# can-lehmann/exprgrad

Measured on AMD Instinct MI355X. Metric: GFLOP/s matmul 4096^3 f32 (1 GPU), higher is better.
Workload: dtype f32

## Files before the change

exprgrad_amd/csrc/kernels/gemm_split_bf16.hip:

```cpp
#include <algorithm>
#include <cfloat>

#include "gemm_fused.hpp"
#include "../eg_internal.hpp"
#include "../switches.hpp"

namespace {

typedef __bf16 bf16x8 __attribute__((ext_vector_type(8)));
typedef float f32x4 __attribute__((ext_vector_type(4)));


struct SplitOperand {
  const float* src;
  long ld;
  long R;
  int kc;
  __bf16* dst;
};

__device__ __forceinline__ void unit_coords(const SplitOperand& o, long K, long u, long& r, long& chunk) {
  const long cpr = K / 8, t = u >> 6;
  const int l = (int)(u & 63);
  if (o.kc) {
    const long per = cpr / 4;
    r = (t / per) * 16 + (l >> 2);
    chunk = (t % per) * 4 + (l & 3);
  } else {
    const long per = cpr / 2;
    r = (t / per) * 32 + (l >> 1);
    chunk = (t % per) * 2 + (l & 1);
  }
}

__device__ __forceinline__ void load_unit(const SplitOperand& o, long r, long chunk, float (&x)[8]) {
  if (o.kc) {
    const f32x4* p = reinterpret_cast<const f32x4*>(o.src + r * o.ld + chunk * 8);
    const f32x4 v0 = __builtin_nontemporal_load(p), v1 = __builtin_nontemporal_load(p + 1);
#pragma unroll
    for (int j = 0; j < 4; ++j) {
      x[j] = v0[j];
      x[4 + j] = v1[j];
    }
  } else {
    const float* p = o.src + chunk * 8 * o.ld + r;
#pragma unroll
    for (int j = 0; j < 8; ++j) x[j] = __builtin_nontemporal_load(p + j * o.ld);
  }
}

__device__ __forceinline__ void split_unit(const SplitOperand& o, long K, long r, long chunk, const float (&x)[8], bool& bad) {
  bf16x8 h0, h1, h2;
#pragma unroll
  for (int j = 0; j < 8; ++j) {
    const float v = x[j];
    const __bf16 b0 = (__bf16)v;
    const float r1 = v - (float)b0;
    const __bf16 b1 = (__bf16)r1;
    const float f1 = (float)b1;
    const float r2 = r1 - f1;
    const __bf16 b2 = (__bf16)r2;
    const float f2 = (float)b2;
    bad |= !(r2 == f2);
    bad |= v != 0.f && __builtin_fabsf(v) < FLT_MIN;
    bad |= (f1 != 0.f && __builtin_fabsf(f1) < FLT_MIN) || (f2 != 0.f && __builtin_fabsf(f2) < FLT_MIN);
    h0[j] = b0;
    h1[j] = b1;
    h2[j] = b2;
  }
  const long plane = o.R * K;
  bf16x8* d = reinterpret_cast<bf16x8*>(o.dst + ((chunk >> 1) * o.R + r) * 16 + (chunk & 1) * 8);
  const long ps = plane / 8;
  d[0] = h0;
  d[ps] = h1;
  d[2 * ps] = h2;
}

constexpr int SPLIT_NT = 256;
constexpr int SPLIT_U = 2;

__global__ __launch_bounds__(SPLIT_NT) void split_planes_kernel(SplitOperand a, SplitOperand b, long K, long units_a, long units,
                                                              unsigned* flag, unsigned epoch) {
  constexpr long STEP = (long)SPLIT_NT * SPLIT_U;
  const long per = ((units + gridDim.x - 1) / gridDim.x + STEP - 1) / STEP * STEP;
  const long lo = (long)blockIdx.x * per, hi = lo + per < units ? lo + per : units;
  bool bad = false;
  for (long base = lo; base < hi; base += STEP) {
    float x[SPLIT_U][8];
    long r[SPLIT_U], c[SPLIT_U];
#pragma unroll
    for (int i = 0; i < SPLIT_U; ++i) {
      const long u = base + i * SPLIT_NT + threadIdx.x;
      if (u >= hi) continue;
      const bool in_a = u < units_a;
      unit_coords(in_a ? a : b, K, in_a ? u : u - units_a, r[i], c[i]);
      load_unit(in_a ? a : b, r[i], c[i], x[i]);
    }
#pragma unroll
    for (int i = 0; i < SPLIT_U; ++i) {
      const long u = base + i * SPLIT_NT + threadIdx.x;
      if (u >= hi) continue;
      split_unit(u < units_a ? a : b, K, r[i], c[i], x[i], bad);
    }
  }
  if (__builtin_expect(bad, 0)) *(volatile unsigned*)flag = epoch;
}


constexpr int BM = 256, BN = 256, WM = 128, WN = 64, NT = 512;
constexpr int STAGES = 3;
constexpr int PLANE_BYTES = BM * 16 * 2;
constexpr int STAGE_BYTES = 6 * PLANE_BYTES;
constexpr int LOADS = STAGE_BYTES / (NT * 16);

struct SplitGemmArgs {
  const __bf16* pa;
  const __bf16* pb;
  float* C;
  const float* bias;
  long M, N, K, ldc;
  int tiles_m, tiles_n;
  int accumulate;
  const unsigned* flag;
  unsigned epoch;
};

__device__ __forceinline__ int xcd_remap(int bid, int nwg) {
  constexpr int NXCD = 8;
  const int q = nwg / NXCD, r = nwg % NXCD;
  const int xcd = bid % NXCD, local = bid / NXCD;
  return (xcd < r ? xcd * (q + 1) : r * (q + 1) + (xcd - r) * q) + local;
}
__device__ __forceinline__ void tile_origin(int wgid, int tiles_m, int tiles_n, long& m_blk, long& n_blk) {
  constexpr int GROUP = 8;
  const int per_group = GROUP * tiles_n;
  const int first_m = (wgid / per_group) * GROUP;
  const int gsize = min(tiles_m - first_m, GROUP);
  const int in_group = wgid % per_group;
  m_blk = (long)(first_m + in_group % gsize) * BM;
  n_blk = (long)(in_group / gsize) * BN;
}

__device__ __forceinline__ const void* uniform_ptr(const void* p) {
  const unsigned long v = reinterpret_cast<unsigned long>(p);
  const unsigned lo = __builtin_amdgcn_readfirstlane((unsigned)v), hi = __builtin_amdgcn_readfirstlane((unsigned)(v >> 32));
  return reinterpret_cast<const void*>(((unsigned long)hi << 32) | lo);
}

__global__ __launch_bounds__(NT) void split_gemm_kernel(SplitGemmArgs a) {
  if (*(volatile const unsigned*)a.flag == a.epoch) return;
  __shared__ __attribute__((aligned(16))) unsigned char lds[STAGES * STAGE_BYTES];

  const int tid = threadIdx.x, lane = tid & 63, wave = tid >> 6;
  const int wr = wave >> 2, wc = wave & 3;
  long m_blk, n_blk;
  tile_origin(xcd_remap(blockIdx.x, gridDim.x), a.tiles_m, a.tiles_n, m_blk, n_blk);

  const __amdgpu_buffer_rsrc_t ra = __builtin_amdgcn_make_buffer_rsrc(
      const_cast<void*>(uniform_ptr(a.pa + m_blk * 16)), (short)0, -1, 0x00020000);
  const __amdgpu_buffer_rsrc_t rb = __builtin_amdgcn_make_buffer_rsrc(
      const_cast<void*>(uniform_ptr(a.pb + n_blk * 16)), (short)0, -1, 0x00020000);
  const unsigned a_plane = (unsigned)(a.M * a.K * 2), b_plane = (unsigned)(a.N * a.K * 2);
  const unsigned a_ktile = (unsigned)(a.M * 32), b_ktile = (unsigned)(a.N * 32);
  const unsigned voff = (unsigned)tid * 16;

  auto issue = [&](int kt, int s) {
    unsigned char* st = lds + s * STAGE_BYTES + wave * 1024;
#pragma unroll
    for (int i = 0; i < LOADS; ++i) {
      __attribute__((address_space(3))) void* dst = (__attribute__((address_space(3))) void*)(st + i * PLANE_BYTES);
      if (i < 3)
        __builtin_amdgcn_raw_ptr_buffer_load_lds(ra, dst, 16, voff, (unsigned)i * a_plane + (unsigned)kt * a_ktile, 0, 0);
      else
        __builtin_amdgcn_raw_ptr_buffer_load_lds(rb, dst, 16, voff, (unsigned)(i - 3) * b_plane + (unsigned)kt * b_ktile, 0, 0);
    }
  };

  f32x4 acc[8][4];
#pragma unroll
  for (int i = 0; i < 8; ++i)
#pragma unroll
    for (int j = 0; j < 4; ++j)
#pragma unroll
      for (int r = 0; r < 4; ++r) acc[i][j][r] = 0.f;

  const int sel = lane >> 5;
  const int a_row = (wr * WM + (lane & 15)) * 32 + ((lane >> 4) & 1) * 16;
  const int b_row = 3 * PLANE_BYTES + (wc * WN + (lane & 15)) * 32 + ((lane >> 4) & 1) * 16;
  const int a01_off = a_row + sel * PLANE_BYTES, a02_off = a_row + 2 * sel * PLANE_BYTES;
  const int b21_off = b_row + (2 - sel) * PLANE_BYTES, b10_off = b_row + (1 - sel) * PLANE_BYTES, b00_off = b_row;

  const int KT = (int)(a.K / 16);
  issue(0, 0);
  if (KT > 1) issue(1, 1);
  int s = 0;
  for (int kt = 0; kt < KT; ++kt) {
    if (kt + 1 < KT) asm volatile("s_waitcnt vmcnt(6)" ::: "memory");
    else asm volatile("s_waitcnt vmcnt(0)" ::: "memory");
    __builtin_amdgcn_s_barrier();
    asm volatile("" ::: "memory");
    if (kt + 2 < KT) issue(kt + 2, s == 0 ? 2 : s - 1);
    const unsigned char* st = lds + s * STAGE_BYTES;
    bf16x8 fb21[4], fb10[4], fb00[4];
#pragma unroll
    for (int j = 0; j < 4; ++j) {
      fb21[j] = *reinterpret_cast<const bf16x8*>(st + b21_off + j * 512);
      fb10[j] = *reinterpret_cast<const bf16x8*>(st + b10_off + j * 512);
      fb00[j] = *reinterpret_cast<const bf16x8*>(st + b00_off + j * 512);
    }
#pragma unroll
    for (int i = 0; i < 8; ++i) {
      const bf16x8 fa01 = *reinterpret_cast<const bf16x8*>(st + a01_off + i * 512);
      const bf16x8 fa02 = *reinterpret_cast<const bf16x8*>(st + a02_off + i * 512);
#pragma unroll
      for (int j = 0; j < 4; ++j) acc[i][j] = __builtin_amdgcn_mfma_f32_16x16x32_bf16(fa01, fb21[j], acc[i][j], 0, 0, 0);
#pragma unroll
      for (int j = 0; j < 4; ++j) acc[i][j] = __builtin_amdgcn_mfma_f32_16x16x32_bf16(fa01, fb10[j], acc[i][j], 0, 0, 0);
#pragma unroll
      for (int j = 0; j < 4; ++j) acc[i][j] = __builtin_amdgcn_mfma_f32_16x16x32_bf16(fa02, fb00[j], acc[i][j], 0, 0, 0);
    }
    s = s == STAGES - 1 ? 0 : s + 1;
  }

  __syncthreads();
  float* park = reinterpret_cast<float*>(lds) + wave * 64 * WN;
  const int prow = lane >> 4, pc4 = (lane & 15) * 4;
  const long col = n_blk + wc * WN + pc4;
  f32x4 b4 = {0.f, 0.f, 0.f, 0.f};
  if (a.bias) b4 = *reinterpret_cast<const f32x4*>(a.bias + col);
#pragma unroll
  for (int h = 0; h < 2; ++h) {
#pragma unroll
    for (int i = 0; i < 4; ++i)
#pragma unroll
      for (int j = 0; j < 4; ++j)
#pragma unroll
        for (int r = 0; r < 4; ++r) park[(i * 16 + 4 * prow + r) * WN + j * 16 + (lane & 15)] = acc[4 * h + i][j][r];
    asm volatile("s_waitcnt lgkmcnt(0)" ::: "memory");
#pragma unroll
    for (int q = 0; q < 16; ++q) {
      const int row = 4 * q + prow;
      f32x4 v = *reinterpret_cast<const f32x4*>(park + row * WN + pc4);
      f32x4* c = reinterpret_cast<f32x4*>(a.C + (m_blk + wr * WM + h * 64 + row) * a.ldc + col);
      if (a.accumulate) v = *c + v;
      if (a.bias) v = v + b4;
      *c = v;
    }
    asm volatile("s_waitcnt lgkmcnt(0)" ::: "memory");
  }
}

inline bool aligned16(const void* p) { return (reinterpret_cast<uintptr_t>(p) & 15) == 0; }

constexpr size_t kPlaneCap = 1ull << 30;

}

namespace eg {
namespace gemm {

int sgemm_split(eg_ctx* ctx, int trans_a, int trans_b, long M, long N, long K, const float* A, long lda, const float* B, long ldb,
                float* C, long ldc, int accumulate, const float* bias) {
  if (!ctx || !A || !B || !C || M <= 0 || N <= 0 || K <= 0) return EG_ERR_UNSUPPORTED;
  if (lda < (trans_a ? M : K) || ldb < (trans_b ? K : N) || ldc < N) return EG_ERR_UNSUPPORTED;
  if (eg::sw::on("EG_NO_SPLIT_GEMM")) return EG_ERR_UNSUPPORTED;
  if (M % BM != 0 || N % BN != 0 || K % 32 != 0 || K < 2048) return EG_ERR_UNSUPPORTED;
  if ((M / BM) * (N / BN) < ctx->compute_units) return EG_ERR_UNSUPPORTED;
  const size_t plane_bytes = 6 * (size_t)(M + N) * (size_t)K;
  if (plane_bytes > kPlaneCap || 6 * (size_t)std::max(M, N) * (size_t)K >= (1ull << 31)) return EG_ERR_UNSUPPORTED;
  if (!aligned16(A) || !aligned16(B) || (!trans_a && lda % 4 != 0) || (trans_b && ldb % 4 != 0)) return EG_ERR_UNSUPPORTED;
  if (!aligned16(C) || ldc % 4 != 0 || (bias && !aligned16(bias))) return EG_ERR_UNSUPPORTED;
  if (!exact_single_launch(ctx, trans_a, trans_b, M, N, K, A, lda, B, ldb, C, ldc, bias)) return EG_ERR_UNSUPPORTED;

  int rc = eg::set_device(ctx);
  if (rc) return rc;
  if (!ctx->split_flag) {
    EG_HIP_CHECK(hipMalloc((void**)&ctx->split_flag, sizeof(unsigned)));
    EG_HIP_CHECK(hipMemset(ctx->split_flag, 0, sizeof(unsigned)));
  }
  rc = eg::ensure_workspace(ctx, plane_bytes);
  if (rc) return rc;
  if (++ctx->split_epoch == 0) ctx->split_epoch = 1;
  const unsigned epoch = ctx->split_epoch;

  __bf16* pa = static_cast<__bf16*>(ctx->workspace);
  __bf16* pb = pa + 3 * (size_t)M * K;
  const SplitOperand oa = {A, lda, M, trans_a ? 0 : 1, pa};
  const SplitOperand ob = {B, ldb, N, trans_b ? 1 : 0, pb};
  const long units_a = M * K / 8, units = (M + N) * K / 8;
  long blocks = (units + SPLIT_NT * SPLIT_U - 1) / (SPLIT_NT * SPLIT_U);
  if (blocks > 8L * ctx->compute_units) blocks = 8L * ctx->compute_units;
  hipLaunchKernelGGL(split_planes_kernel, dim3((unsigned)blocks), dim3(SPLIT_NT), 0, ctx->stream, oa, ob, K, units_a, units,
                     ctx->split_flag, epoch);
  EG_HIP_CHECK(hipGetLastError());

  SplitGemmArgs g = {};
  g.pa = pa;
  g.pb = pb;
  g.C = C;
  g.bias = bias;
  g.M = M;
  g.N = N;
  g.K = K;
  g.ldc = ldc;
  g.tiles_m = (int)(M / BM);
  g.tiles_n = (int)(N / BN);
  g.accumulate = accumulate;
  g.flag = ctx->split_flag;
  g.epoch = epoch;
  hipLaunchKernelGGL(split_gemm_kernel, dim3((unsigned)(g.tiles_m * g.tiles_n)), dim3(NT), 0, ctx->stream, g);
  EG_HIP_CHECK(hipGetLastError());

  return sgemm_exact(ctx, trans_a, trans_b, M, N, K, A, lda, B, ldb, C, ldc, accumulate, bias, ctx->split_flag, epoch);
}

}
}
```

Before: 238,400.

## Specialize wave roles in split-bf16 GEMM: half the waves load, others prefetch fragments

Adds a skew mode, on by default. Waves with bit 2 set issue the global-to-LDS loads for themselves and their partner wave. The other waves issue no loads and read the next stage's B and A-head fragments at the end of each iteration, which staggers LDS reads against MFMA work across waves. The A fragment loads inside the inner loop are also software-pipelined one row ahead, and the wave index is forced to be scalar. Skew mode waits for vmcnt(0) every iteration, which may expose load latency, and an optional timestamp instrumentation path is compiled in under a macro.

```diff
diff --git a/exprgrad_amd/csrc/kernels/gemm_split_bf16.hip b/exprgrad_amd/csrc/kernels/gemm_split_bf16.hip
--- a/exprgrad_amd/csrc/kernels/gemm_split_bf16.hip
+++ b/exprgrad_amd/csrc/kernels/gemm_split_bf16.hip
@@ -121,6 +121,7 @@
   long M, N, K, ldc;
   int tiles_m, tiles_n;
   int accumulate;
+  int skew;
   const unsigned* flag;
   unsigned epoch;
 };
@@ -147,11 +148,29 @@
   return reinterpret_cast<const void*>(((unsigned long)hi << 32) | lo);
 }
 
+constexpr int ROLE_LOAD_OWN = 1, ROLE_LOAD_PARTNER = 2, ROLE_READ_TOP = 4, ROLE_READ_AHEAD = 8;
+constexpr int PARTNER = 4;
+
+#ifdef EG_SPLIT_GEMM_STAMPS
+constexpr int STAMP_BLOCKS = 1024;
+__device__ unsigned long long g_split_stamps[STAMP_BLOCKS][8][4];
+#define EG_STAMP(t)                                                                  \
+  do {                                                                               \
+    __builtin_amdgcn_sched_barrier(0);                                               \
+    asm volatile("s_memtime %0\n\ts_waitcnt lgkmcnt(0)" : "=s"(t)::"memory"); \
+    __builtin_amdgcn_sched_barrier(0);                                               \
+  } while (0)
+#else
+#define EG_STAMP(t) \
+  do {              \
+  } while (0)
+#endif
+
 __global__ __launch_bounds__(NT) void split_gemm_kernel(SplitGemmArgs a) {
   if (*(volatile const unsigned*)a.flag == a.epoch) return;
   __shared__ __attribute__((aligned(16))) unsigned char lds[STAGES * STAGE_BYTES];
 
-  const int tid = threadIdx.x, lane = tid & 63, wave = tid >> 6;
+  const int tid = threadIdx.x, lane = tid & 63, wave = __builtin_amdgcn_readfirstlane(tid >> 6);
   const int wr = wave >> 2, wc = wave & 3;
   long m_blk, n_blk;
   tile_origin(xcd_remap(blockIdx.x, gridDim.x), a.tiles_m, a.tiles_n, m_blk, n_blk);
@@ -162,18 +181,23 @@
       const_cast<void*>(uniform_ptr(a.pb + n_blk * 16)), (short)0, -1, 0x00020000);
   const unsigned a_plane = (unsigned)(a.M * a.K * 2), b_plane = (unsigned)(a.N * a.K * 2);
   const unsigned a_ktile = (unsigned)(a.M * 32), b_ktile = (unsigned)(a.N * 32);
-  const unsigned voff = (unsigned)tid * 16;
-
-  auto issue = [&](int kt, int s) {
-    unsigned char* st = lds + s * STAGE_BYTES + wave * 1024;
+  const unsigned voff = (unsigned)lane * 16;
+
+  auto pieces = [&](int kt, int s, int w) {
+    unsigned char* st = lds + s * STAGE_BYTES + w * 1024;
+    const unsigned at = (unsigned)kt * a_ktile + (unsigned)w * 1024, bt = (unsigned)kt * b_ktile + (unsigned)w * 1024;
 #pragma unroll
     for (int i = 0; i < LOADS; ++i) {
       __attribute__((address_space(3))) void* dst = (__attribute__((address_space(3))) void*)(st + i * PLANE_BYTES);
       if (i < 3)
-        __builtin_amdgcn_raw_ptr_buffer_load_lds(ra, dst, 16, voff, (unsigned)i * a_plane + (unsigned)kt * a_ktile, 0, 0);
+        __builtin_amdgcn_raw_ptr_buffer_load_lds(ra, dst, 16, voff, (unsigned)i * a_plane + at, 0, 0);
       else
-        __builtin_amdgcn_raw_ptr_buffer_load_lds(rb, dst, 16, voff, (unsigned)(i - 3) * b_plane + (unsigned)kt * b_ktile, 0, 0);
-    }
+        __builtin_amdgcn_raw_ptr_buffer_load_lds(rb, dst, 16, voff, (unsigned)(i - 3) * b_plane + bt, 0, 0);
+    }
+  };
+  auto issue = [&](int kt, int s, int r) {
+    if (r & ROLE_LOAD_OWN) pieces(kt, s, wave);
+    if (r & ROLE_LOAD_PARTNER) pieces(kt, s, wave ^ PARTNER);
   };
 
   f32x4 acc[8][4];
@@ -190,37 +214,89 @@
   const int a01_off = a_row + sel * PLANE_BYTES, a02_off = a_row + 2 * sel * PLANE_BYTES;
   const int b21_off = b_row + (2 - sel) * PLANE_BYTES, b10_off = b_row + (1 - sel) * PLANE_BYTES, b00_off = b_row;
 
-  const int KT = (int)(a.K / 16);
-  issue(0, 0);
-  if (KT > 1) issue(1, 1);
-  int s = 0;
-  for (int kt = 0; kt < KT; ++kt) {
-    if (kt + 1 < KT) asm volatile("s_waitcnt vmcnt(6)" ::: "memory");
-    else asm volatile("s_waitcnt vmcnt(0)" ::: "memory");
-    __builtin_amdgcn_s_barrier();
-    asm volatile("" ::: "memory");
-    if (kt + 2 < KT) issue(kt + 2, s == 0 ? 2 : s - 1);
-    const unsigned char* st = lds + s * STAGE_BYTES;
-    bf16x8 fb21[4], fb10[4], fb00[4];
+  bf16x8 fb21[4], fb10[4], fb00[4], fa01, fa02;
+  auto read_head = [&](const unsigned char* st) {
 #pragma unroll
     for (int j = 0; j < 4; ++j) {
       fb21[j] = *reinterpret_cast<const bf16x8*>(st + b21_off + j * 512);
       fb10[j] = *reinterpret_cast<const bf16x8*>(st + b10_off + j * 512);
       fb00[j] = *reinterpret_cast<const bf16x8*>(st + b00_off + j * 512);
     }
+    fa01 = *reinterpret_cast<const bf16x8*>(st + a01_off);
+    fa02 = *reinterpret_cast<const bf16x8*>(st + a02_off);
+  };
+#pragma unroll
+  for (int j = 0; j < 4; ++j) fb21[j] = fb10[j] = fb00[j] = bf16x8{};
+  fa01 = fa02 = bf16x8{};
+
+  const int skew = a.skew;
+  const int role = !skew ? ROLE_LOAD_OWN | ROLE_READ_TOP
+                         : (wave & PARTNER) ? ROLE_LOAD_OWN | ROLE_LOAD_PARTNER | ROLE_READ_TOP : ROLE_READ_AHEAD;
+  const int KT = (int)(a.K / 16);
+  issue(0, 0, role);
+  if (KT > 1) issue(1, 1, role);
+  if (skew) {
+    if (KT > 1) asm volatile("s_waitcnt vmcnt(12)" ::: "memory");
+    else asm volatile("s_waitcnt vmcnt(0)" ::: "memory");
+    __builtin_amdgcn_s_barrier();
+    asm volatile("" ::: "memory");
+    if (role & ROLE_READ_AHEAD) read_head(lds);
+  }
+#ifdef EG_SPLIT_GEMM_STAMPS
+  unsigned long long t0 = 0, t1 = 0, t2 = 0, front = 0, body = 0, back = 0;
+#endif
+  int s = 0;
+  for (int kt = 0; kt < KT; ++kt) {
+    if (!skew && kt + 1 < KT) asm volatile("s_waitcnt vmcnt(6)" ::: "memory");
+    else asm volatile("s_waitcnt vmcnt(0)" ::: "memory");
+    __builtin_amdgcn_s_barrier();
+    asm volatile("" ::: "memory");
+#ifdef EG_SPLIT_GEMM_STAMPS
+    EG_STAMP(t0);
+    if (kt) back += t0 - t2;
+#endif
+    int r = role;
+    asm volatile("" : "+s"(r));
+    if (kt + 2 < KT) issue(kt + 2, s == 0 ? 2 : s - 1, r);
+    const unsigned char* st = lds + s * STAGE_BYTES;
+    if (r & ROLE_READ_TOP) read_head(st);
+    EG_STAMP(t1);
+    bf16x8 c01 = fa01, c02 = fa02;
 #pragma unroll
     for (int i = 0; i < 8; ++i) {
-      const bf16x8 fa01 = *reinterpret_cast<const bf16x8*>(st + a01_off + i * 512);
-      const bf16x8 fa02 = *reinterpret_cast<const bf16x8*>(st + a02_off + i * 512);
-#pragma unroll
-      for (int j = 0; j < 4; ++j) acc[i][j] = __builtin_amdgcn_mfma_f32_16x16x32_bf16(fa01, fb21[j], acc[i][j], 0, 0, 0);
-#pragma unroll
-      for (int j = 0; j < 4; ++j) acc[i][j] = __builtin_amdgcn_mfma_f32_16x16x32_bf16(fa01, fb10[j], acc[i][j], 0, 0, 0);
-#pragma unroll
-      for (int j = 0; j < 4; ++j) acc[i][j] = __builtin_amdgcn_mfma_f32_16x16x32_bf16(fa02, fb00[j], acc[i][j], 0, 0, 0);
-    }
+      bf16x8 n01 = c01, n02 = c02;
+      __builtin_amdgcn_sched_barrier(0);
+      if (i + 1 < 8) {
+        n01 = *reinterpret_cast<const bf16x8*>(st + a01_off + (i + 1) * 512);
+        n02 = *reinterpret_cast<const bf16x8*>(st + a02_off + (i + 1) * 512);
+      }
+      __builtin_amdgcn_sched_barrier(0);
+#pragma unroll
+      for (int j = 0; j < 4; ++j) acc[i][j] = __builtin_amdgcn_mfma_f32_16x16x32_bf16(c01, fb21[j], acc[i][j], 0, 0, 0);
+#pragma unroll
+      for (int j = 0; j < 4; ++j) acc[i][j] = __builtin_amdgcn_mfma_f32_16x16x32_bf16(c01, fb10[j], acc[i][j], 0, 0, 0);
+#pragma unroll
+      for (int j = 0; j < 4; ++j) acc[i][j] = __builtin_amdgcn_mfma_f32_16x16x32_bf16(c02, fb00[j], acc[i][j], 0, 0, 0);
+      c01 = n01;
+      c02 = n02;
+    }
+    EG_STAMP(t2);
+#ifdef EG_SPLIT_GEMM_STAMPS
+    front += t1 - t0;
+    body += t2 - t1;
+#endif
     s = s == STAGES - 1 ? 0 : s + 1;
-  }
+    if ((r & ROLE_READ_AHEAD) && kt + 1 < KT) read_head(lds + s * STAGE_BYTES);
+  }
+#ifdef EG_SPLIT_GEMM_STAMPS
+  if (lane == 0 && blockIdx.x < STAMP_BLOCKS) {
+    unsigned long long* o = g_split_stamps[blockIdx.x][wave];
+    o[0] = front;
+    o[1] = body;
+    o[2] = back;
+    o[3] = (unsigned long long)KT;
+  }
+#endif
 
   __syncthreads();
   float* park = reinterpret_cast<float*>(lds) + wave * 64 * WN;
@@ -306,6 +382,7 @@
   g.tiles_m = (int)(M / BM);
   g.tiles_n = (int)(N / BN);
   g.accumulate = accumulate;
+  g.skew = eg::sw::present("EG_GEMM_NO_SKEW") ? 0 : 1;
   g.flag = ctx->split_flag;
   g.epoch = epoch;
   hipLaunchKernelGGL(split_gemm_kernel, dim3((unsigned)(g.tiles_m * g.tiles_n)), dim3(NT), 0, ctx->stream, g);
@@ -316,3 +393,12 @@
 
 }
 }
+
+#ifdef EG_SPLIT_GEMM_STAMPS
+extern "C" int eg_debug_split_stamps(unsigned long long* dst, size_t count) {
+  if (count > sizeof(g_split_stamps) / sizeof(unsigned long long)) return EG_ERR_UNSUPPORTED;
+  EG_HIP_CHECK(hipDeviceSynchronize());
+  EG_HIP_CHECK(hipMemcpyFromSymbol(dst, HIP_SYMBOL(g_split_stamps), count * sizeof(unsigned long long)));
+  return 0;
+}
+#endif
```

Result: faster. 249,400, median of 6 (+4.6%).
